# jonathanventura/spherical-sfm

Hardware: AMD Instinct MI355X
Metric: BA obs/sec (Jac+Schur+PCG) (higher is better)
Workload: dtype f64; 1 GPU; 300 cams x 100000 pts x 600000 obs synthetic circle (BASELINE configs[1]), general BA, focal fixed, CauchyLoss(1.0), Ceres-default LM; camera_dof=6, comm=none, reduced_solver=band-cholesky (direct), pcg_sweeps=0

## Files before the change

spherical_sfm_amd/csrc/ba_handle.h:

```cpp
#pragma once
#include <atomic>
#include <hip/hip_runtime.h>
#include <chrono>
#include <cmath>
#include <cstring>
#include <limits>
#include <string>
#include <vector>
#include "ba_flatten.h"
#include "ba_kernels.h"
#include "band_kernels2.h"
#include "band_kernels2p.h"
#include "band_sub.h"
#include "band_ring.h"
#include "snode.h"
#include "ssfm_ctx.h"
#include "knobs.h"

namespace ssfm {

static double wall_s() { return std::chrono::duration<double>(std::chrono::steady_clock::now().time_since_epoch()).count(); }

enum KernelId { KID_CAM_ROT, KID_POINT_LIN, KID_SCHUR_ROWS, KID_FINALIZE, KID_PCG_INIT, KID_PCG_MATVEC, KID_PCG_VECOPS,
                KID_CAM_UPDATE, KID_BACKSUB, KID_COST, KID_ALLREDUCE, KID_BAND_GATHER, KID_BAND_CHOL, KID_BAND_FWD, KID_BAND_BACK,
// ... 39 lines not shown

struct ssfm_ba_handle {
    ssfm_ctx* ctx = nullptr;
    int device = 0;
    ssfm_ba_options opt;
    BAFlat F;
    int n_red = 0;
    DevBuf<double> cam_x, cam_c, cam_init, pts_x, pts_c, pts_init, focal3;
    DevBuf<double> rot_x, rot_c, scale_cam, scale_pt, scale_f, mask_cam, mask_pt, mask_f, diag_cam, diag_pt, diag_f;
    DevBuf<double> obs_xy; DevBuf<int> obs_cam, obs_pt, pt_start, cam_start, cam_obs, row_ptr, col_idx, diag_slot;
    DevBuf<double> zone; bool zone_views = false; size_t zone_len = 0, zone_nnz = 0, zone_n = 0;
    bool det = false; DevBuf<long long> det_limb, det_lacc; DevBuf<double> det_dfpart; size_t det_nacc = 0;
    static constexpr size_t det_lacc_words = (size_t)SC_NSLOT * SC_TOTAL * LA_STRIDE;
    hipError_t clear_det_lacc() { return hipMemsetAsync(det_lacc.p, 0, det_lacc_words * sizeof(long long), ctx->stream); }
    void set_zone(int which) {
        scal.p = zone.p + (size_t)which * zone_len; pcg.p = scal.p + scal.n; redbuf.p = pcg.p + pcg.n;
        S_val = redbuf.p; rhs = S_val + zone_nnz; Udiag = rhs + (zone_n + 1); Sfc = Udiag + zone_n; gcraw = Sfc + zone_n; red_scal = gcraw + zone_n;
    }
    DevBuf<double> lmdev;
    DevBuf<double> Vs, gp, redbuf, Minv, Sff, px, pr, pz, pp, pq, pqpart, scal, pcg;
    DevBuf<double> band, Linv, Yb, Yr; DevBuf<int> cam_pos, band_pairs, band_fail, comp_ptr;
    BandSub sub; DevBuf<int> sub_seg_lo, sub_seg_hi, sub_seg_wend, sub_left, sub_sep_lo, sub_sep_rseg, sub_chain_ptr, sub_tw_lo, sub_tw_hi, sub_tw_copy, sub_seg_given, sub_seg_mode;
    DevBuf<unsigned char> pair_dummy;
    DevBuf<int> cam_pos2;
    DevBuf<double> subZ, subD, subT, subF, subL, subW, subC, subTc; DevBuf<int> sub_flags, sub_fz_lo, sub_fz_hi, sub_fz_wend, sub_fz_merge, sub_fz_await, sub_fz_signal, sub_fz_flags; int sub_seq = 0, sub_fz_seq = 0;
    DevBuf<int> col_pos, trans_pos;
    DevBuf<int> wrap_ptr, wrap_blk, wrap_row2, ring_rec, ring_tail; DevBuf<double> crL, crF, crW, crP, crT, crE;
    const int* wrap_ptr_p() const { return wrap_ptr.n ? wrap_ptr.p : nullptr; }
    SnodePlan sn; DevBuf<int> sn_half, sn_step, sn_node, sn_tab, sn_flags; DevBuf<double> sn_work, sn_xchg; int sn_seq = 0;
    DevBuf<int> trans_ptr, trans_blk, trans_row, pair_j, pair_j2, pair_p, batch_slot, cam_batch_ptr, chunk_cam, chunk_b0, chunk_b1, cam_obs_pt, cs_task_cam, cs_task_q0, cs_task_q1;
    double *S_val = nullptr, *rhs = nullptr, *Udiag = nullptr, *Sfc = nullptr, *gcraw = nullptr, *red_scal = nullptr;
    double focal_host = 0, t_flatten_s = 0;
    double* host_sp = nullptr;
    double* host_pub = nullptr;
    bool scale_ready = false;
    bool band_filled = false;
    struct { bool on = false, residual_later = false; const double *cam = nullptr, *focal = nullptr; double *cam_c = nullptr, *focal_c = nullptr, *rot_c = nullptr; } tail;
    DevBuf<int> gr_rec; DevBuf<unsigned char> pt_grouped;
    DevBuf<double> gram_part; DevBuf<int> gpart_off, fold_slot_ptr, fold_slot_src; bool gram_fold = false;
    DevBuf<int> pub_ticket;
    int pcg_prev_iters = 16;
    bool external_tail = false;
    bool profile = false;
    std::vector<hipEvent_t> ev_pool; size_t ev_used = 0;
    struct Span { int kid; hipEvent_t a, b; };
    std::vector<Span> spans;
    int64_t k_launches[KID_COUNT]; double k_ms[KID_COUNT];
    hipEvent_t phase_ev[5] = {nullptr, nullptr, nullptr, nullptr, nullptr};
    hipEvent_t x0_ev = nullptr;

    hipEvent_t get_event() {
        if (ev_used == ev_pool.size()) { hipEvent_t e; (void)hipEventCreate(&e); ev_pool.push_back(e); }
        return ev_pool[ev_used++];
    }
    void span_begin(int kid) { if (!profile) return; Span s{kid, get_event(), get_event()}; (void)hipEventRecord(s.a, ctx->stream); spans.push_back(s); }
    void span_end() { if (!profile) return; (void)hipEventRecord(spans.back().b, ctx->stream); }
    void resolve_spans() {
        for (auto& s : spans) { float ms = 0; if (hipEventElapsedTime(&ms, s.a, s.b) == hipSuccess) { k_ms[s.kid] += ms; k_launches[s.kid]++; } }
        spans.clear(); ev_used = 0;
    }
    void free_all() {
        cam_x.free(); cam_c.free(); cam_init.free(); pts_x.free(); pts_c.free(); pts_init.free(); focal3.free();
        rot_x.free(); rot_c.free(); scale_cam.free(); scale_pt.free(); scale_f.free(); mask_cam.free(); mask_pt.free(); mask_f.free();
        diag_cam.free(); diag_pt.free(); diag_f.free(); obs_xy.free(); obs_cam.free(); obs_pt.free(); pt_start.free();
        cam_start.free(); cam_obs.free(); row_ptr.free(); col_idx.free(); diag_slot.free(); Vs.free(); gp.free();
        lmdev.free(); band.free(); Linv.free(); Yb.free(); Yr.free(); cam_pos.free(); band_pairs.free(); band_fail.free(); comp_ptr.free();
        sub_seg_lo.free(); sub_seg_hi.free(); sub_seg_wend.free(); sub_left.free(); sub_sep_lo.free(); sub_sep_rseg.free(); sub_chain_ptr.free(); sub_tw_lo.free(); sub_tw_hi.free(); sub_tw_copy.free(); sub_seg_given.free(); sub_seg_mode.free(); cam_pos2.free(); pair_dummy.free();
        subZ.free(); subD.free(); subT.free(); subF.free(); subL.free(); subW.free(); subC.free(); subTc.free(); sub_flags.free(); sub_fz_lo.free(); sub_fz_hi.free(); sub_fz_wend.free(); sub_fz_merge.free(); sub_fz_await.free(); sub_fz_signal.free(); sub_fz_flags.free();
        col_pos.free(); trans_pos.free(); trans_ptr.free(); trans_blk.free(); trans_row.free(); pair_j.free(); pair_j2.free(); pair_p.free(); batch_slot.free(); cam_batch_ptr.free(); chunk_cam.free(); chunk_b0.free(); chunk_b1.free(); cam_obs_pt.free(); cs_task_cam.free(); cs_task_q0.free(); cs_task_q1.free();
        if (zone_views) { scal.p = nullptr; pcg.p = nullptr; redbuf.p = nullptr; zone_views = false; }
        pub_ticket.free(); gr_rec.free(); pt_grouped.free();
        gram_part.free(); gpart_off.free(); fold_slot_ptr.free(); fold_slot_src.free(); gram_fold = false;
        sn_half.free(); sn_step.free(); sn_node.free(); sn_tab.free(); sn_flags.free(); sn_work.free(); sn_xchg.free(); sn.enabled = false;
        wrap_ptr.free(); wrap_blk.free(); wrap_row2.free(); ring_rec.free(); ring_tail.free(); crL.free(); crF.free(); crW.free(); crP.free(); crT.free(); crE.free();
        zone.free(); redbuf.free(); Minv.free(); Sff.free(); px.free(); pr.free(); pz.free(); pp.free(); pq.free(); pqpart.free(); scal.free(); pcg.free();
        if (host_sp) { (void)hipHostFree(host_sp); host_sp = nullptr; }
        host_pub = nullptr;
        for (auto e : ev_pool) (void)hipEventDestroy(e);
        ev_pool.clear();
        for (auto& e : phase_ev) if (e) { (void)hipEventDestroy(e); e = nullptr; }
        if (x0_ev) { (void)hipEventDestroy(x0_ev); x0_ev = nullptr; }
    }
};

namespace ssfm {

#define MATVEC(h, DCV, vec)                                                                                                   \
    do {                                                                                                                   \
        if ((h)->F.sym_lower)                                                                                              \
            LAUNCH(h, KID_PCG_MATVEC, k_sym_matvec<DCV>, ((h)->F.Nc + 3) / 4, 256, 0, (h)->row_ptr.p, (h)->col_idx.p, (h)->trans_ptr.p, \
// ... 84 lines not shown
}
static int wait_published(ssfm_ba_handle* h) {
    ssfm_ctx* ctx = h->ctx;
    volatile unsigned long long* flag = reinterpret_cast<volatile unsigned long long*>(h->host_pub + SC_TOTAL + PCG_TOTAL + 1);
    const unsigned long long want = ctx->pub_seq;
    unsigned spins = 0;
    while (*flag != want) {
        cpu_relax();
        if ((++spins & 0xFFFFu) == 0) {
            const hipError_t q = hipStreamQuery(ctx->stream);
            if (q == hipSuccess) { if (*flag == want) break; return fail(ctx, SSFM_ERR_HIP, "an LM iteration ended without publishing its scalars"); }
            if (q != hipErrorNotReady) return fail(ctx, SSFM_ERR_HIP, hipGetErrorString(q));
        }
    }
    std::atomic_thread_fence(std::memory_order_acquire);
    return SSFM_OK;
}

static int sub_upload(ssfm_ba_handle* h, int DC) {
    ssfm_ctx* ctx = h->ctx; hipStream_t st = ctx->stream; const BAFlat& F = h->F;
    if (F.band_block > 0) DC = F.band_block;
    sub_build(F.comp_ptr, F.comp_twist, F.band, DC, h->sub, &F.rings);
    if (!F.wrap_ptr.empty()) { SSFM_HIP_CHECK(ctx, upload(h->wrap_ptr, F.wrap_ptr, st)); SSFM_HIP_CHECK(ctx, upload(h->wrap_blk, F.wrap_blk, st)); SSFM_HIP_CHECK(ctx, upload(h->wrap_row2, F.wrap_row2, st)); }
    if (!h->sub.enabled) return SSFM_OK;
    const BandSub& B = h->sub; const size_t Q = (size_t)F.band * DC, n = (size_t)(F.band_rows > 0 ? F.band_rows : F.Nc) * DC;
    SSFM_HIP_CHECK(ctx, upload(h->sub_tw_lo, B.tw_lo, st)); SSFM_HIP_CHECK(ctx, upload(h->sub_tw_hi, B.tw_hi, st)); SSFM_HIP_CHECK(ctx, upload(h->sub_tw_copy, B.tw_copy, st)); SSFM_HIP_CHECK(ctx, upload(h->sub_seg_given, B.seg_given, st));
    {
        std::vector<int> mode(B.seg_twist.size());
        for (size_t i = 0; i < mode.size(); i++) mode[i] = B.seg_twist[i] >= 0 ? 1 + (B.seg_twist[i] & 1) : 0;
        SSFM_HIP_CHECK(ctx, upload(h->sub_seg_mode, mode, st));
    }
    SSFM_HIP_CHECK(ctx, upload(h->sub_seg_lo, B.seg_lo, st)); SSFM_HIP_CHECK(ctx, upload(h->sub_seg_hi, B.seg_hi, st));
    SSFM_HIP_CHECK(ctx, upload(h->sub_seg_wend, B.seg_wend, st)); SSFM_HIP_CHECK(ctx, upload(h->sub_left, B.left_segs, st));
    SSFM_HIP_CHECK(ctx, upload(h->sub_sep_lo, B.sep_lo, st)); SSFM_HIP_CHECK(ctx, upload(h->sub_sep_rseg, B.sep_rseg, st));
    SSFM_HIP_CHECK(ctx, upload(h->sub_chain_ptr, B.chain_ptr, st));
    if (B.ntwist > 0) {
        SSFM_HIP_CHECK(ctx, upload(h->sub_fz_lo, B.fz_lo, st)); SSFM_HIP_CHECK(ctx, upload(h->sub_fz_hi, B.fz_hi, st)); SSFM_HIP_CHECK(ctx, upload(h->sub_fz_wend, B.fz_wend, st));
        SSFM_HIP_CHECK(ctx, upload(h->sub_fz_merge, B.fz_merge, st)); SSFM_HIP_CHECK(ctx, upload(h->sub_fz_await, B.fz_await, st)); SSFM_HIP_CHECK(ctx, upload(h->sub_fz_signal, B.fz_signal, st));
        SSFM_HIP_CHECK(ctx, h->sub_fz_flags.alloc((size_t)4 * B.ntwist)); SSFM_HIP_CHECK(ctx, hipMemsetAsync(h->sub_fz_flags.p, 0, (size_t)4 * B.ntwist * sizeof(int), st)); h->sub_fz_seq = 0;
    }
    if (B.nsep == 0) return SSFM_OK;
    SSFM_HIP_CHECK(ctx, h->subZ.alloc(Q * n)); SSFM_HIP_CHECK(ctx, h->subD.alloc((size_t)B.nsep * Q * Q)); SSFM_HIP_CHECK(ctx, h->subT.alloc((size_t)B.nsep * 2 * Q));
    SSFM_HIP_CHECK(ctx, h->subF.alloc((size_t)(B.nsep + B.nchain) * Q * Q)); SSFM_HIP_CHECK(ctx, h->subL.alloc((size_t)B.nsep * Q * (Q + 1) / 2)); SSFM_HIP_CHECK(ctx, h->subW.alloc((size_t)B.nsep * 2 * Q));
    SSFM_HIP_CHECK(ctx, h->subC.alloc((size_t)B.nchain * Q * (Q + 1) / 2)); SSFM_HIP_CHECK(ctx, h->subTc.alloc((size_t)B.nchain * 2 * Q)); SSFM_HIP_CHECK(ctx, h->sub_flags.alloc((size_t)2 * B.nchain));
    SSFM_HIP_CHECK(ctx, hipMemsetAsync(h->sub_flags.p, 0, (size_t)2 * B.nchain * sizeof(int), st)); h->sub_seq = 0;
    if (B.nring > 0) {
// ... 194 lines not shown
                    if (lb > 48 * 1024) SSFM_HIP_CHECK(ctx, hipFuncSetAttribute(reinterpret_cast<const void*>(k_ring_cr_back<DC, 2>), hipFuncAttributeMaxDynamicSharedMemorySize, (int)lb));
                    if (lt > 48 * 1024) SSFM_HIP_CHECK(ctx, hipFuncSetAttribute(reinterpret_cast<const void*>(k_ring_cr_tail<DC, 2>), hipFuncAttributeMaxDynamicSharedMemorySize, (int)lt));
                    const int nsteps = (int)B.ring_step_ptr.size() - 1;
                    const int cr_threads = Q > 48 ? 1024 : 512;
                    static int ring_stamp_state = SSFM_LAB_KNOB("SSFM_RING_STAMPS", 0) ? 1 : 0; static long long* ring_stamps = nullptr;
                    if (ring_stamp_state == 1) { (void)hipMalloc((void**)&ring_stamps, (size_t)4 * B.nsep * sizeof(long long)); (void)hipMemsetAsync(ring_stamps, 0, (size_t)4 * B.nsep * sizeof(long long), st); ring_stamp_state = 2; }
                    for (int sidx = 0; sidx < nsteps; sidx++)
                        LAUNCH(h, KID_RING_ELIM, (k_ring_cr_elim<DC, 2>), dim3(B.ring_step_ptr[sidx + 1] - B.ring_step_ptr[sidx], elim_roles(B.ring_step_ptr[sidx + 1] - B.ring_step_ptr[sidx])), cr_threads, le, h->ring_rec.p, B.ring_step_ptr[sidx], h->subZ.p, h->subD.p, h->subT.p,
                               h->crL.p, h->crF.p, h->crW.p, h->crP.p, h->crT.p, h->crE.p, Nc, b, failp, ring_stamp_state == 2 ? ring_stamps : (long long*)nullptr);
                    if (ring_stamp_state == 2) {
                        std::vector<long long> hs((size_t)4 * B.nsep); (void)hipStreamSynchronize(st); (void)hipMemcpy(hs.data(), ring_stamps, hs.size() * sizeof(long long), hipMemcpyDeviceToHost);
                        double a = 0, bb = 0, c = 0; int cnt = 0;
                        for (int q = 0; q < B.nsep; q++) if (hs[4 * q + 3] > 0) { a += hs[4 * q + 1] - hs[4 * q]; bb += hs[4 * q + 2] - hs[4 * q + 1]; c += hs[4 * q + 3] - hs[4 * q + 2]; cnt++; }
                        if (cnt) std::fprintf(stderr, "[ring stamps, 100 MHz ticks] Q = %d, %d eliminations (parallel steps): loads %.0f | factorisation %.0f | stores + neighbour products %.0f\n", Q, cnt, a / cnt, bb / cnt, c / cnt);
                        (void)hipFree(ring_stamps); ring_stamps = nullptr; ring_stamp_state = 3;
                    }
                    LAUNCH(h, KID_RING_TAIL, (k_ring_cr_tail<DC, 2>), B.nring, cr_threads, lt, h->ring_rec.p, h->ring_tail.p, h->subZ.p, h->subD.p, h->subT.p,
                           h->crL.p, h->crF.p, h->crW.p, h->crP.p, h->crT.p, h->crE.p, Y, Nc, b, failp);
                    for (int sidx = nsteps - 1; sidx >= 0; sidx--)
                        LAUNCH(h, KID_RING_BACK, (k_ring_cr_back<DC, 2>), B.ring_step_ptr[sidx + 1] - B.ring_step_ptr[sidx], back_threads, lb, h->ring_rec.p, B.ring_step_ptr[sidx], h->crL.p, h->crF.p, h->crW.p, Y, Nc, b);
                }
            }
            static const bool back_fuse = SSFM_LAB_KNOB("SSFM_BACK_FUSE", 0) != 0;
            if (B.ntwist > 0) {
                if (wide2p) SSFM_LAUNCH_CHOL2P(B.ntwist, h->sub_tw_lo.p, h->sub_tw_hi.p, h->sub_tw_hi.p, h->sub_tw_copy.p);
                else if (!fused) SSFM_LAUNCH_CHOL2(B.ntwist, h->band.p, h->Linv.p, Y, h->band_pairs.p, h->sub_tw_lo.p, h->sub_tw_hi.p, h->sub_tw_hi.p, h->sub_tw_copy.p, Nc, b, failp, chol_map);
                if (!back_fuse) {
                h->span_begin(KID_BAND_BACK);
                BACK_V2_LAUNCH(dim3(B.ntwist, 2), h->band.p, h->Linv.p, Y, h->sub_tw_lo.p, h->sub_tw_hi.p, h->sub_tw_hi.p, (const int*)nullptr, Nc, b);
                h->span_end();
                }
            }
            if (B.nleft > 0) {
                h->span_begin(KID_SUB_APPLY);
                hipLaunchKernelGGL((k_sub_apply_left<DC, 2>), dim3(B.nleft, (max_rows + APPLY_ROWS - 1) / APPLY_ROWS), dim3(APPLY_ROWS * APPLY_SLICES), (size_t)(2 * Q + APPLY_SLICES * APPLY_ROWS * 2) * sizeof(double), st, h->subZ.p, Y, h->sub_seg_lo.p, h->sub_seg_hi.p, h->sub_left.p, Nc, b);
                h->span_end();
            }
            h->span_begin(KID_BAND_BACK);
            BACK_V2_LAUNCH(dim3(B.nseg, 2), h->band.p, h->Linv.p, Y, h->sub_seg_lo.p, h->sub_seg_hi.p, h->sub_seg_wend.p, h->sub_seg_given.p, Nc, b, (const int*)(back_fuse ? h->sub_seg_mode.p : nullptr));
            h->span_end();
            return SSFM_OK;
        }
        if (wide2p) {
            SSFM_LAUNCH_CHOL2P(ncomp, h->comp_ptr.p, h->comp_ptr.p + 1, h->comp_ptr.p + 1, (const int*)nullptr);
            h->span_begin(KID_BAND_BACK);
            BACK_V2_LAUNCH(dim3(ncomp, 2), h->band.p, h->Linv.p, Y, h->comp_ptr.p, h->comp_ptr.p + 1, h->comp_ptr.p + 1, (const int*)nullptr, Nc, b);
            h->span_end();
        } else if (use_lds) {
            SSFM_LAUNCH_CHOL2(ncomp, h->band.p, h->Linv.p, Y, h->band_pairs.p, h->comp_ptr.p, h->comp_ptr.p + 1, h->comp_ptr.p + 1, (const int*)nullptr, Nc, b, reinterpret_cast<int*>(h->pcg.p + PCG_TOTAL), chol_map);
            if (back_v2) {
                h->span_begin(KID_BAND_BACK);
                BACK_V2_LAUNCH(dim3(ncomp, 2), h->band.p, h->Linv.p, Y, h->comp_ptr.p, h->comp_ptr.p + 1, h->comp_ptr.p + 1, (const int*)nullptr, Nc, b);
                h->span_end();
            } else {
                LAUNCH(h, KID_BAND_BACK, (k_band_back_lds<DC, 2>), ncomp, 256, lds_sub2, h->band.p, h->Linv.p, Y, h->comp_ptr.p, Nc, b);
            }
        } else {
            LAUNCH(h, KID_BAND_CHOL, (k_band_chol<DC, 2>), 1, 1024, lds_chol, h->band.p, h->Linv.p, Y, h->band_pairs.p, Nc, b, reinterpret_cast<int*>(h->pcg.p + PCG_TOTAL));
            LAUNCH(h, KID_BAND_BACK, (k_band_back<DC, 2>), 1, 256, lds_sub2, h->band.p, h->Linv.p, Y, Nc, b);
        }
        return SSFM_OK;
#undef SSFM_LAUNCH_CHOL2
#undef SSFM_LAUNCH_CHOL2_V
#undef SSFM_LAUNCH_CHOL2P
#undef SSFM_LAUNCH_2P
#undef SSFM_LAUNCH_2P6
    }

template <int DC>
static int band_resolve(ssfm_ba_handle* h, double* Y, bool* needs_refactor) {
    hipStream_t st = h->ctx->stream;
    const BAFlat& F = h->F;
// ... 114 lines not shown
```

spherical_sfm_amd/csrc/ba_solver.hip:

```cpp
#include <atomic>
#include <hip/hip_runtime.h>
#include <chrono>
#include <cmath>
#include <cstdlib>
#include <cstring>
#include <limits>
#include <string>
#include <vector>
#include "ba_flatten.h"
#include "ba_kernels.h"
#include "band_kernels.h"
#include "knobs.h"
#include "ssfm_ctx.h"

#include "ba_handle.h"

namespace ssfm {

constexpr unsigned DET_K_ASSEMBLY = (1u << SC_COST) | (1u << SC_FJJ) | (1u << SC_FJR) | (1u << SC_FWW) | (1u << SC_FWG);
constexpr unsigned DET_K_TAIL = (1u << SC_MODEL) | (1u << SC_STEP2_PT) | (1u << SC_XN2_PT) | (1u << SC_CAND_COST) | (1u << SC_STEP2_CAM) | (1u << SC_XN2_CAM);
static unsigned det_tail_mask(bool with_cams, bool gram_fold) {
    const unsigned tail = with_cams ? (DET_K_TAIL & ~((1u << SC_STEP2_CAM) | (1u << SC_XN2_CAM))) : DET_K_TAIL;
    return tail | (gram_fold ? (1u << SC_COST) : 0u);
}
// ... 62 lines not shown
            double* host_sp = h->host_sp;
            for (int k = 0; k < SC_TOTAL; k++) {
                double a = host_sp[k];
                for (int s2 = 1; s2 < SC_NSLOT; s2++) { const double v = host_sp[(size_t)s2 * SC_TOTAL + k]; a = (k == SC_GMAX) ? std::max(a, v) : a + v; }
                host_sp[k] = a;
            }
        }
        return SSFM_OK;
    }
    int need_x0() {
        if (!x0_pending) return SSFM_OK;
        SSFM_HIP_CHECK(ctx, hipEventSynchronize(h->x0_ev));
        x_norm = std::sqrt(host_scal[SC_X0N2_PT] + host_scal[SC_X0N2_CAM]); x0_pending = false;
        return SSFM_OK;
    }

    int read_knobs() {
        poll = lm_poll() && publish_alloc(h);
        if (!poll && !h->host_sp) SSFM_HIP_CHECK(ctx, hipHostMalloc((void**)&h->host_sp, (SC_NSLOT * SC_TOTAL + PCG_TOTAL + 1) * sizeof(double), hipHostMallocDefault));
        host_scal = poll ? h->host_pub : h->host_sp; host_pcg1 = poll ? h->host_pub + SC_TOTAL : h->host_sp + SC_NSLOT * SC_TOTAL;
        spec_on = poll && nP > 0 && knob_env_int("SSFM_LM_SPECULATE", 1) != 0;
        gram_bs = knob_env_int("SSFM_GRAM_BACKSUB", -1);
        gbs_split_env = knob_env_int("SSFM_GBS_SPLIT", 0);
        fuse_lin = SSFM_LAB_KNOB("SSFM_GRAM_FUSE", 0) != 0 && nP > 0 && !F.gr_rec.empty() && F.gram_points == (int64_t)nP && F.chunk_cam.empty() && F.cs_task_cam.empty();
        return SSFM_OK;
    }

    int startup() {
        { const int rc = read_knobs(); if (rc) return rc; }
        const int gp_pts = (nP + 255) / 256;
        h->set_zone(0);
        if (h->det) {
            if (!h->gram_fold) SSFM_HIP_CHECK(ctx, hipMemsetAsync(h->det_limb.p, 0, (2 * h->det_nacc + 2) * sizeof(long long), st));
            SSFM_HIP_CHECK(ctx, h->clear_det_lacc());
        }
        const bool make_scale = !h->scale_ready;
        LAUNCH(h, KID_CAM_ROT, k_cam_rot0, gp_cam, 64, 0, x.cam, x.rot, Nc, h->scal.p, (int)SC_TOTAL, h->diag_f.p, make_scale ? 1 : 0);
        if (make_scale) {
            if (nP > 0) hipLaunchKernelGGL(k_colnorm_both, dim3(gp_pts + Nc), dim3(256), 0, st, gp_pts, x.cam, x.rot, x.pts, x.focal, oxy, h->obs_cam.p, h->pt_start.p, nP,
                                           loss, la, h->diag_pt.p, h->diag_f.p, h->mask_pt.p, h->scale_pt.p, O.jacobi_scaling, h->det ? h->det_dfpart.p : (double*)nullptr,
                                           h->obs_pt.p, h->cam_start.p, h->cam_obs.p, h->diag_cam.p, h->mask_cam.p, ctx->collective ? (double*)nullptr : h->scale_cam.p);
            else hipLaunchKernelGGL(k_colnorm_cam, dim3(Nc), dim3(256), 0, st, x.cam, x.rot, x.pts, x.focal, oxy, h->obs_pt.p, h->cam_start.p, h->cam_obs.p,
                               loss, la, h->diag_cam.p, h->mask_cam.p, ctx->collective ? (double*)nullptr : h->scale_cam.p, O.jacobi_scaling);
            if (ctx->collective) {
                int rc = allreduce(h, h->diag_cam.p, (size_t)Nc * 6, ncclSum); if (rc) return rc;
                rc = allreduce(h, h->diag_f.p, 1, ncclSum); if (rc) return rc;
// ... 378 lines not shown
}

extern "C" int ssfm_band_solve_probe(ssfm_ctx* ctx, int32_t dc, int32_t N, int32_t b, int32_t ncomp, const int32_t* comp_ptr, const double* band,
                                     double* Y, int32_t* segs_seps_fail, double* Zdump, double* Ddump, double* Tdump) {
    if (!ctx || (dc != 3 && dc != 6) || N <= 0 || b < 1 || ncomp < 1 || !comp_ptr || !band || !Y) return fail(ctx, SSFM_ERR_INVALID, "ssfm_band_solve_probe: bad arguments");
    SSFM_HIP_CHECK(ctx, hipSetDevice(ctx->device));
    hipStream_t st = ctx->stream;
    ssfm_ba_handle hh; ssfm_ba_handle* h = &hh;
    h->ctx = ctx; ssfm_ba_default_options(&h->opt);
    std::memset(h->k_launches, 0, sizeof(h->k_launches)); std::memset(h->k_ms, 0, sizeof(h->k_ms));
    BAFlat& F = h->F; F.Nc = N; F.band_rows = N; F.band_block = dc; F.band = b; F.DC = dc; F.comp_ptr.assign(comp_ptr, comp_ptr + ncomp + 1);
    for (int ir = 1; ir <= b; ir++) for (int kr = 1; kr <= ir; kr++) F.band_pairs.push_back(ir | (kr << 16));
    const size_t nb = (size_t)N * (b + 1) * dc * dc, n = (size_t)N * dc;
    int rc = SSFM_OK;
    auto run = [&]() -> int {
        SSFM_HIP_CHECK(ctx, h->band.alloc(nb)); SSFM_HIP_CHECK(ctx, h->Linv.alloc((size_t)N * dc * dc)); SSFM_HIP_CHECK(ctx, h->Yb.alloc(2 * n));
        SSFM_HIP_CHECK(ctx, h->pcg.alloc(PCG_TOTAL + 1));
        SSFM_HIP_CHECK(ctx, hipMemsetAsync(h->pcg.p, 0, (PCG_TOTAL + 1) * sizeof(double), st));
        SSFM_HIP_CHECK(ctx, hipMemsetAsync(h->Linv.p, 0, (size_t)N * dc * dc * sizeof(double), st));
        SSFM_HIP_CHECK(ctx, hipMemcpyAsync(h->band.p, band, nb * sizeof(double), hipMemcpyHostToDevice, st));
        SSFM_HIP_CHECK(ctx, hipMemcpyAsync(h->Yb.p, Y, 2 * n * sizeof(double), hipMemcpyHostToDevice, st));
        SSFM_HIP_CHECK(ctx, upload(h->band_pairs, F.band_pairs, st)); SSFM_HIP_CHECK(ctx, upload(h->comp_ptr, F.comp_ptr, st));
        { const int r = sub_upload(h, dc); if (r) return r; }
        if (h->sub.enabled && h->subZ.p) SSFM_HIP_CHECK(ctx, hipMemsetAsync(h->subZ.p, 0, h->subZ.n * sizeof(double), st));
        { const int r = (dc == 3) ? band_direct<3>(h, h->Yb.p) : band_direct<6>(h, h->Yb.p); if (r) return r; }
        SSFM_HIP_CHECK(ctx, hipMemcpyAsync(Y, h->Yb.p, 2 * n * sizeof(double), hipMemcpyDeviceToHost, st));
        int flag = 0;
        SSFM_HIP_CHECK(ctx, hipMemcpyAsync(&flag, h->pcg.p + PCG_TOTAL, sizeof(int), hipMemcpyDeviceToHost, st));
        if (h->sub.enabled) {
            if (Zdump) SSFM_HIP_CHECK(ctx, hipMemcpyAsync(Zdump, h->subZ.p, h->subZ.n * sizeof(double), hipMemcpyDeviceToHost, st));
            if (Ddump) SSFM_HIP_CHECK(ctx, hipMemcpyAsync(Ddump, h->subD.p, h->subD.n * sizeof(double), hipMemcpyDeviceToHost, st));
            if (Tdump) SSFM_HIP_CHECK(ctx, hipMemcpyAsync(Tdump, h->subT.p, h->subT.n * sizeof(double), hipMemcpyDeviceToHost, st));
        }
        SSFM_HIP_CHECK(ctx, hipStreamSynchronize(st));
        if (segs_seps_fail) { segs_seps_fail[0] = h->sub.enabled ? h->sub.nseg : ncomp; segs_seps_fail[1] = h->sub.nsep; segs_seps_fail[2] = flag; }
        return SSFM_OK;
    };
    rc = run();
    h->free_all();
    return rc;
}


extern "C" int ssfm_snode_solve_probe(ssfm_ctx* ctx, int32_t dc, int32_t Nc, const int32_t* row_ptr, const int32_t* col_idx, const double* S_val, const double* rhs2,
                                      int32_t nr, double* Y, int32_t* info) {
    if (!ctx || (dc != 3 && dc != 6) || Nc <= 0 || !row_ptr || !col_idx || !S_val || !rhs2 || !Y || !info || (nr != 1 && nr != 2)) return fail(ctx, SSFM_ERR_INVALID, "ssfm_snode_solve_probe: bad arguments");
// ... 507 lines not shown
```

spherical_sfm_amd/csrc/band_kernels2.h:

```cpp
#pragma once
#include <type_traits>
#include "band_kernels.h"

namespace ssfm {

__device__ __forceinline__ double lane_bcast(double v, int src_lane) {
    const int lo = __builtin_amdgcn_readlane(__double2loint(v), src_lane), hi = __builtin_amdgcn_readlane(__double2hiint(v), src_lane);
    return __hiloint2double(hi, lo);
}
__device__ __forceinline__ double lane_shift_down(double v, int delta) {
    const int idx = (int)(((threadIdx.x & 63) + delta) & 63) << 2;
    const int lo = __builtin_amdgcn_ds_bpermute(idx, __double2loint(v)), hi = __builtin_amdgcn_ds_bpermute(idx, __double2hiint(v));
    return __hiloint2double(hi, lo);
}

template <int DC>
__device__ __forceinline__ bool wave_chol_inverse(double (&row)[DC], double (&g)[DC]) {
    const int lane = threadIdx.x & 63;
    double L[DC], rs[DC]; bool ok = true;
#pragma unroll
    for (int c = 0; c < DC; c++) {
        double d = lane_bcast(row[c], c);
        ok = ok && (d > 0.0);
        rs[c] = fast_rsqrt(d);
// ... 19 lines not shown
    if (nw != 9) return m;
    int weight[16], order[16];
    for (int r = 0; r < nw; r++) {
        weight[r] = (r == 0) ? 12 : (r <= ntw) ? ((r <= heavy_tw) ? 6 : 2) : (r == nw - 1) ? 5 : 4;
        order[r] = r;
    }
    for (int a = 0; a < nw; a++) for (int c = a + 1; c < nw; c++) if (weight[order[c]] > weight[order[a]]) { const int t = order[a]; order[a] = order[c]; order[c] = t; }
    int load[4] = {0, 0, 0, 0}, used[4] = {0, 0, 0, 0}, cap[4];
    for (int q = 0; q < 4; q++) cap[q] = (nw - q + 3) / 4;
    bool placed[16] = {false};
    m.v[0] = (unsigned char)order[0]; placed[0] = true; used[0] = 1;
    for (int a = nw - 1; a >= 1 && used[0] < cap[0]; a--) { m.v[4 * used[0]] = (unsigned char)order[a]; placed[a] = true; used[0]++; }
    for (int a = 1; a < nw; a++) {
        if (placed[a]) continue;
        int best = -1;
        for (int q = 1; q < 4; q++) if (used[q] < cap[q] && (best < 0 || load[q] < load[best])) best = q;
        m.v[best + 4 * used[best]] = (unsigned char)order[a];
        load[best] += weight[order[a]]; used[best]++;
    }
    return m;
}

constexpr int BACK_PD = 4;
template <int DC, int NS, bool to_lds, bool from_lds>
__device__ __forceinline__ void band_back_sweep(const double* __restrict__ band, const double* __restrict__ Ginv, double* __restrict__ y, double* xs,
                                                const int r0, const int r1, const int re, const int gf, const int b, const int lane) {
    constexpr int BB = DC * DC;
    const int W = b + 1, T = b * DC;
    int dd[NS], off[NS]; bool has[NS];
#pragma unroll
    for (int s = 0; s < NS; s++) {
        const int t = min(lane + 64 * s, T - 1);
        dd[s] = t / DC + 1; off[s] = dd[s] * BB + (t - (dd[s] - 1) * DC); has[s] = lane + 64 * s < T;
    }
    const int lc = min(lane, DC - 1);
    struct Stage { double col[NS][DC], li[DC], yv; };
    const size_t row_stride = (size_t)W * BB;
        Stage st[BACK_PD];
        auto fetch = [&](int j, Stage& s) {
            const int jc = max(j, r0);
            const double* __restrict__ rowp = band + (size_t)jc * row_stride;
            const double* __restrict__ gpt = Ginv + (size_t)jc * BB;
#pragma unroll
            for (int m = 0; m < DC; m++) {
#pragma unroll
                for (int q = 0; q < NS; q++) s.col[q][m] = rowp[off[q] + m * DC];
                s.li[m] = gpt[m * DC + lc];
            }
            const int jy = (gf >= 0 && jc >= r1) ? gf + (re - 1 - jc) : jc;
            s.yv = (from_lds && jc >= r1) ? xs[(jy - gf) * DC + lc] : y[(size_t)jy * DC + lc];
        };
#pragma unroll
        for (int u = 0; u < BACK_PD; u++) fetch(re - 1 - u, st[u]);
        double acc[NS];
#pragma unroll
        for (int q = 0; q < NS; q++) acc[q] = 0.0;
        for (int jb = re - 1; jb >= r0; jb -= BACK_PD) {
#pragma unroll
            for (int u = 0; u < BACK_PD; u++) {
                const int j = jb - u;
                if (j < r0) break;
                double c[NS][DC], cl[DC]; const double cy = st[u].yv;
                bool v[NS];
#pragma unroll
                for (int q = 0; q < NS; q++) v[q] = has[q] && j - dd[q] >= r0;
#pragma unroll
                for (int m = 0; m < DC; m++) {
#pragma unroll
                    for (int q = 0; q < NS; q++) c[q][m] = st[u].col[q][m];
                    cl[m] = st[u].li[m];
                }
                fetch(j - BACK_PD, st[u]);
                const double z = cy - acc[0];
                double sh[NS], sft[NS];
#pragma unroll
                for (int q = 0; q < NS; q++) sh[q] = lane_shift_down(acc[q], DC);
#pragma unroll
                for (int q = 0; q < NS; q++) {
                    const double next = (q + 1 < NS) ? sh[q + 1 < NS ? q + 1 : q] : 0.0;
                    sft[q] = (lane + DC < 64) ? sh[q] : next;
                    if (!(lane + 64 * q + DC < T)) sft[q] = 0.0;
                }
                double x = 0.0;
#pragma unroll
                for (int k = 0; k < DC; k++) x += cl[k] * lane_bcast(z, k);
                if (j >= r1) x = cy;
                else if (lane < DC) { if (to_lds) xs[(j - r0) * DC + lane] = x; else y[(size_t)j * DC + lane] = x; }
                double sm[NS];
#pragma unroll
                for (int q = 0; q < NS; q++) sm[q] = 0.0;
#pragma unroll
                for (int m = 0; m < DC; m++) { const double xm = lane_bcast(x, m);
#pragma unroll
                    for (int q = 0; q < NS; q++) sm[q] += c[q][m] * xm; }
#pragma unroll
                for (int q = 0; q < NS; q++) acc[q] = sft[q] + (v[q] ? sm[q] : 0.0);
            }
        }
}

template <int DC, int NR, int MF = 0, int TCW = 3>
__global__ void __launch_bounds__(768)
k_band_chol_v2(double* __restrict__ band, double* __restrict__ Ginv, double* __restrict__ Y, const int* __restrict__ pairs,
               const int* __restrict__ piv_lo, const int* __restrict__ piv_hi, const int* __restrict__ win_hi,
               const int* __restrict__ merge_from, int N, int b, int* __restrict__ fail_flag,
               const CholWaveMap wmap,
               const int* __restrict__ await2 = nullptr, const int* __restrict__ signal = nullptr, int* __restrict__ flags = nullptr, int seq = 0) {
    constexpr int BB = DC * DC;
    extern __shared__ __attribute__((aligned(16))) double lds[];
    const int R = b + 1, W = b + 1, RW = W * BB;
    double* sWin = lds;
    double* sP = sWin + (size_t)R * RW;
    double* sYr = sP + (size_t)b * BB;
    double* sYj = sYr + (size_t)R * NR * DC;
    double* sG = sYj + NR * DC;
    double* sD = sG + BB;
    int* sPairs = reinterpret_cast<int*>(sD + BB);
    const int n = N * DC, nt = blockDim.x, lane = threadIdx.x & 63, nw = nt >> 6;
    const int wave = __builtin_amdgcn_readfirstlane((int)wmap.v[threadIdx.x >> 6]), tid = wave * 64 + lane;
    const int ntw = nw - 2 - CHOL2_LOADERS;
    const int r0 = piv_lo[blockIdx.x], r1 = piv_hi[blockIdx.x], re = win_hi[blockIdx.x];
    const int sig = signal ? signal[blockIdx.x] : -1, aw = await2 ? await2[blockIdx.x] : -1;
    if (r0 >= r1) { if (sig >= 0 && tid == 0) __hip_atomic_store(flags + sig, seq, __ATOMIC_RELEASE, __HIP_MEMORY_SCOPE_AGENT); return; }
    for (int e = tid; e < b * (b + 1) / 2; e += nt) sPairs[e] = pairs[e];
    if (aw >= 0) {
        if (tid == 0) { while (__hip_atomic_load(flags + aw, __ATOMIC_ACQUIRE, __HIP_MEMORY_SCOPE_AGENT) != seq) __builtin_amdgcn_s_sleep(8);
                        while (__hip_atomic_load(flags + aw + 1, __ATOMIC_ACQUIRE, __HIP_MEMORY_SCOPE_AGENT) != seq) __builtin_amdgcn_s_sleep(8); }
        __syncthreads(); __threadfence();
    }
    const int mf = merge_from ? merge_from[blockIdx.x] : -1;
// ... 363 lines not shown
#undef CHOL2_ISSUE
#undef CHOL2_STEP
    } else {
        int jm = jm0;
        for (int j = r0; j < r1; j++, jm = (jm + 1 == R) ? 0 : jm + 1) {
            const int nb = min(b, re - 1 - j);
            phaseB(j, jm, nb);
            for (int e = lane; e < BB; e += 64) Ginv[(size_t)j * BB + e] = sG[e];
            lds_barrier();
            for (int e = lane; e < nb * BB; e += 64) { const int k = e / BB; band[((size_t)(j + 1 + k) * W + (k + 1)) * BB + (e - k * BB)] = sP[e]; }
            if (lane < NR * DC) Y[(size_t)(lane / DC) * n + (size_t)j * DC + (lane % DC)] = sYj[lane];
            lds_barrier();
        }
    }
    if (re > r1) {
        __syncthreads();
        for (int row = r1; row < re; row++) {
            const int nin = (row - r1 + 1) * BB;
            const double* src = sWin + (size_t)(row % R) * RW;
            for (int e = tid; e < nin; e += nt) band[(size_t)row * RW + e] = src[e];
            for (int e = tid; e < NR * DC; e += nt) Y[(size_t)(e / DC) * n + (size_t)row * DC + (e % DC)] = sYr[(size_t)(row % R) * NR * DC + e];
        }
    }
    if (sig >= 0) {
        __threadfence(); __syncthreads();
        if (tid == 0) __hip_atomic_store(flags + sig, seq, __ATOMIC_RELEASE, __HIP_MEMORY_SCOPE_AGENT);
    }
}

template <int DC, int NS>
__global__ void __launch_bounds__(64)
k_band_back_v2(const double* __restrict__ band, const double* __restrict__ Ginv, double* __restrict__ Y, const int* __restrict__ piv_lo,
               const int* __restrict__ piv_hi, const int* __restrict__ win_hi, const int* __restrict__ given_from, int N, int b,
               const int* __restrict__ tw_mode = nullptr) {
    __shared__ double xs[32 * DC];
    const int n = N * DC, lane = threadIdx.x;
    const int mode = tw_mode ? tw_mode[blockIdx.x] : 0;
    if (piv_lo[blockIdx.x] >= piv_hi[blockIdx.x]) return;
    double* y = Y + (size_t)blockIdx.y * n;
    const int r0 = piv_lo[blockIdx.x], r1 = piv_hi[blockIdx.x], re = win_hi[blockIdx.x];
    const int gf = given_from ? given_from[blockIdx.x] : -1;
    if (mode == 2) {
        band_back_sweep<DC, NS, true, false>(band, Ginv, y, xs, gf, gf + b, gf + b, -1, b, lane);
        __builtin_amdgcn_fence(__ATOMIC_RELEASE, "wavefront"); __builtin_amdgcn_fence(__ATOMIC_ACQUIRE, "wavefront");
        band_back_sweep<DC, NS, false, true>(band, Ginv, y, xs, r0, r1, re, gf, b, lane);
    } else band_back_sweep<DC, NS, false, false>(band, Ginv, y, xs, r0, mode == 1 ? re : r1, re, mode == 1 ? -1 : gf, b, lane);
// ... 4 lines not shown
```

spherical_sfm_amd/csrc/rotavg_solver.hip:

```cpp
#include <algorithm>
#include <cstdio>
#include "ba_handle.h"
#include "dual.h"
#include "line_search.h"

namespace ssfm {

struct EdgeConst { double meas[9]; double r[3]; double rx, ry, thetaxy, thetaz; };

static void decompose_rotation_host(const double* R, double& rx, double& ry, double& thetaxy, double& thetaz) {
    double Z[3] = {R[2], R[5], R[8]};
    const double zn = norm3(Z); Z[0] /= zn; Z[1] /= zn; Z[2] /= zn;
    const double axis[3] = {-Z[1], Z[0], 0.0};
    const double an = norm3(axis);
    const double rxy[3] = {axis[0] / an, axis[1] / an, axis[2] / an};
    thetaxy = acos(Z[2]);
    const double v[3] = {thetaxy * rxy[0], thetaxy * rxy[1], thetaxy * rxy[2]};
    double Rxy[9]; so3exp(v, Rxy);
    rx = rxy[0]; ry = rxy[1];
    double Rz[9]; mat3_mul_at(Rxy, R, Rz);
    double rz[3]; so3ln(Rz, rz);
    thetaz = rz[2];
}

// ... 574 lines not shown
        }
        std::vector<int> nptr(n + 1, 0), nedge, nslot; std::vector<unsigned char> nside, nfirst;
        for (int i = 0; i < n; i++) {
            auto& v = adj[i];
            std::sort(v.begin(), v.end(), [](const Ent& p, const Ent& q) { return p.nb != q.nb ? p.nb < q.nb : p.e < q.e; });
            for (size_t k = 0; k < v.size(); k++) {
                nedge.push_back(v[k].e); nside.push_back(v[k].side);
                nslot.push_back((int)(std::lower_bound(F.col_idx.begin() + F.row_ptr[i], F.col_idx.begin() + F.row_ptr[i + 1], v[k].nb) - (F.col_idx.begin() + F.row_ptr[i])));
                nfirst.push_back((k == 0 || v[k - 1].nb != v[k].nb) ? 1 : 0);
            }
            nptr[i + 1] = (int)nedge.size();
        }
        if (nedge.empty()) { nedge.push_back(0); nslot.push_back(0); nside.push_back(0); nfirst.push_back(0); }
        std::vector<int> zero2(2, 0);
        SSFM_HIP_CHECK(ctx, su.up(RS.nadj_ptr, nptr)); SSFM_HIP_CHECK(ctx, su.up(RS.nadj_edge, nedge)); SSFM_HIP_CHECK(ctx, su.up(RS.nadj_slot, nslot));
        SSFM_HIP_CHECK(ctx, su.up(RS.nadj_side, nside)); SSFM_HIP_CHECK(ctx, su.up(RS.nadj_first, nfirst)); SSFM_HIP_CHECK(ctx, su.up(RS.ticket, zero2));
        ALV(RS.ejac, (size_t)24 * E); ALV(RS.node_part, (size_t)3 * ((E + 63) / 64)); ALV(RS.wg_part, (size_t)5 * ((E + 63) / 64 + gnode)); ALV(RS.step_part, (size_t)5 * 32);
    }
#undef ALV
    double* fmx = fm2.p; double* fmc = fm2.p + 1; double* xx = x.p; double* xcand = xc.p;
    const int ge = (E + 63) / 64, gn = (n + 63) / 64;
    const double la = O.loss_scale;
    const bool poll = lm_poll() && publish_alloc(h);
    if (!poll && !h->host_sp) SSFM_HIP_CHECK(ctx, hipHostMalloc((void**)&h->host_sp, (SC_NSLOT * SC_TOTAL + PCG_TOTAL + 1) * sizeof(double), hipHostMallocDefault));
    double* host_scal = poll ? h->host_pub : h->host_sp; double* host_pcg = poll ? h->host_pub + SC_TOTAL : h->host_sp + SC_NSLOT * SC_TOTAL;
    SSFM_HIP_CHECK(ctx, hipMemsetAsync(h->zone.p, 0, h->zone.n * sizeof(double), st));
    auto assemble = [&](const double* s3, const double* sf) -> int {
        if (node_major) {
            hipLaunchKernelGGL(k_rot_edge_records, dim3(ge), dim3(64), 0, st, kind, E, e0.p, e1.p, ec.p, G.scale, la, xx, fmx, s3, sf, RS.ejac.p, RS.node_part.p);
            hipLaunchKernelGGL(k_rot_gather_nodes, dim3(n), dim3(64), 0, st, n, ge, RS.nadj_ptr.p, RS.nadj_edge.p, RS.nadj_side.p, RS.nadj_slot.p, RS.nadj_first.p, RS.ejac.p, RS.node_part.p,
                               h->row_ptr.p, h->diag_slot.p, h->S_val, h->rhs, h->Udiag, h->Sfc, h->scal.p, h->pcg.p + PCG_TOTAL);
        } else
        hipLaunchKernelGGL(k_rot_edges, dim3(ge), dim3(64), 0, st, 0, kind, E, e0.p, e1.p, ec.p, G.scale, la, xx, fmx, s3, sf, h->row_ptr.p, h->col_idx.p, n,
                           (const double*)nullptr, h->S_val, h->rhs, h->Udiag, h->Sfc, h->scal.p);
        return SSFM_OK;
    };
    {
        DevBuf<double>&m3 = RS.m3, &mf = RS.mf; std::vector<double> mfv = {with_f ? 1.0 : 0.0};
        SSFM_HIP_CHECK(ctx, su.up(m3, G.mask)); SSFM_HIP_CHECK(ctx, su.up(mf, mfv));
        int rc = assemble(m3.p, mf.p); if (rc) return rc;
        hipLaunchKernelGGL(k_make_scale, dim3((3 * n + 255) / 256), dim3(256), 0, st, h->Udiag, m3.p, sc3.p, 3 * n, O.jacobi_scaling);
        hipLaunchKernelGGL(k_make_scale, dim3(1), dim3(64), 0, st, h->scal.p + SC_FJJ, mf.p, scf.p, 1, O.jacobi_scaling);
        hipLaunchKernelGGL(k_scale3to6, dim3((6 * n + 255) / 256), dim3(256), 0, st, sc3.p, n, sc6.p);
        if (timing) SSFM_HIP_CHECK(ctx, hipStreamSynchronize(st));
    }
    lap("allocations, uploads, Jacobi scaling");
// ... 154 lines not shown
```

Baseline: 3.565 billion obs/s.

## Fuse band back-substitution into the Cholesky kernel tail

Adds a per-component or per-twist record table and runs the banded back-substitution sweeps at the end of the LDS Cholesky kernel, instead of launching a separate back-sweep kernel. Idle waves prefetch the band and Ginv segments into cache while the main sweep runs, and the back sweep uses a configurable prefetch depth. This removes one kernel launch and the band re-read from the per-LM-iteration direct solve. In exchange it adds extra barriers and a serial back sweep inside the Cholesky workgroup, and it only applies under specific segment layouts.

```diff
diff --git a/spherical_sfm_amd/csrc/ba_handle.h b/spherical_sfm_amd/csrc/ba_handle.h
--- a/spherical_sfm_amd/csrc/ba_handle.h
+++ b/spherical_sfm_amd/csrc/ba_handle.h
@@ -85,6 +85,7 @@
     DevBuf<double> band, Linv, Yb, Yr; DevBuf<int> cam_pos, band_pairs, band_fail, comp_ptr;
     BandSub sub; DevBuf<int> sub_seg_lo, sub_seg_hi, sub_seg_wend, sub_left, sub_sep_lo, sub_sep_rseg, sub_chain_ptr, sub_tw_lo, sub_tw_hi, sub_tw_copy, sub_seg_given, sub_seg_mode;
     DevBuf<unsigned char> pair_dummy;
+    DevBuf<int> back_rec; bool back_in_chol = true;
     DevBuf<int> cam_pos2;
     DevBuf<double> subZ, subD, subT, subF, subL, subW, subC, subTc; DevBuf<int> sub_flags, sub_fz_lo, sub_fz_hi, sub_fz_wend, sub_fz_merge, sub_fz_await, sub_fz_signal, sub_fz_flags; int sub_seq = 0, sub_fz_seq = 0;
     DevBuf<int> col_pos, trans_pos;
@@ -128,7 +129,7 @@
         diag_cam.free(); diag_pt.free(); diag_f.free(); obs_xy.free(); obs_cam.free(); obs_pt.free(); pt_start.free();
         cam_start.free(); cam_obs.free(); row_ptr.free(); col_idx.free(); diag_slot.free(); Vs.free(); gp.free();
         lmdev.free(); band.free(); Linv.free(); Yb.free(); Yr.free(); cam_pos.free(); band_pairs.free(); band_fail.free(); comp_ptr.free();
-        sub_seg_lo.free(); sub_seg_hi.free(); sub_seg_wend.free(); sub_left.free(); sub_sep_lo.free(); sub_sep_rseg.free(); sub_chain_ptr.free(); sub_tw_lo.free(); sub_tw_hi.free(); sub_tw_copy.free(); sub_seg_given.free(); sub_seg_mode.free(); cam_pos2.free(); pair_dummy.free();
+        sub_seg_lo.free(); sub_seg_hi.free(); sub_seg_wend.free(); sub_left.free(); sub_sep_lo.free(); sub_sep_rseg.free(); sub_chain_ptr.free(); sub_tw_lo.free(); sub_tw_hi.free(); sub_tw_copy.free(); sub_seg_given.free(); sub_seg_mode.free(); back_rec.free(); cam_pos2.free(); pair_dummy.free();
         subZ.free(); subD.free(); subT.free(); subF.free(); subL.free(); subW.free(); subC.free(); subTc.free(); sub_flags.free(); sub_fz_lo.free(); sub_fz_hi.free(); sub_fz_wend.free(); sub_fz_merge.free(); sub_fz_await.free(); sub_fz_signal.free(); sub_fz_flags.free();
         col_pos.free(); trans_pos.free(); trans_ptr.free(); trans_blk.free(); trans_row.free(); pair_j.free(); pair_j2.free(); pair_p.free(); batch_slot.free(); cam_batch_ptr.free(); chunk_cam.free(); chunk_b0.free(); chunk_b1.free(); cam_obs_pt.free(); cs_task_cam.free(); cs_task_q0.free(); cs_task_q1.free();
         if (zone_views) { scal.p = nullptr; pcg.p = nullptr; redbuf.p = nullptr; zone_views = false; }
@@ -259,6 +260,16 @@
     if (F.band_block > 0) DC = F.band_block;
     sub_build(F.comp_ptr, F.comp_twist, F.band, DC, h->sub, &F.rings);
     if (!F.wrap_ptr.empty()) { SSFM_HIP_CHECK(ctx, upload(h->wrap_ptr, F.wrap_ptr, st)); SSFM_HIP_CHECK(ctx, upload(h->wrap_blk, F.wrap_blk, st)); SSFM_HIP_CHECK(ctx, upload(h->wrap_row2, F.wrap_row2, st)); }
+    {
+        const BandSub& Bs = h->sub;
+        const int nrec = Bs.enabled ? Bs.ntwist : (int)F.comp_ptr.size() - 1;
+        std::vector<int> rec((size_t)BACK_REC_INTS * std::max(nrec, 0), 0);
+        if (Bs.enabled) for (int sg = 0; sg < Bs.nseg; sg++) if (Bs.seg_twist[sg] >= 0) {
+            int* r = rec.data() + (size_t)BACK_REC_INTS * (Bs.seg_twist[sg] >> 1) + 4 * (Bs.seg_twist[sg] & 1);
+            r[0] = Bs.seg_lo[sg]; r[1] = Bs.seg_hi[sg]; r[2] = Bs.seg_wend[sg]; r[3] = Bs.seg_given[sg];
+        }
+        if (nrec > 0) SSFM_HIP_CHECK(ctx, upload(h->back_rec, rec, st));
+    }
     if (!h->sub.enabled) return SSFM_OK;
     const BandSub& B = h->sub; const size_t Q = (size_t)F.band * DC, n = (size_t)(F.band_rows > 0 ? F.band_rows : F.Nc) * DC;
     SSFM_HIP_CHECK(ctx, upload(h->sub_tw_lo, B.tw_lo, st)); SSFM_HIP_CHECK(ctx, upload(h->sub_tw_hi, B.tw_hi, st)); SSFM_HIP_CHECK(ctx, upload(h->sub_tw_copy, B.tw_copy, st)); SSFM_HIP_CHECK(ctx, upload(h->sub_seg_given, B.seg_given, st));
@@ -499,6 +510,12 @@
                 }
             }
             static const bool back_fuse = SSFM_LAB_KNOB("SSFM_BACK_FUSE", 0) != 0;
+            const bool back_in = h->back_in_chol && b * DC <= 64 && !wide2p && !fused && !back_fuse && B.ntwist > 0 && B.nsep == 0 && B.nleft == 0 && B.nseg == 2 * B.ntwist && h->back_rec.p;
+            if (back_in) {
+                SSFM_LAUNCH_CHOL2(B.ntwist, h->band.p, h->Linv.p, Y, h->band_pairs.p, h->sub_tw_lo.p, h->sub_tw_hi.p, h->sub_tw_hi.p, h->sub_tw_copy.p, Nc, b, failp, chol_map,
+                                  (const int*)nullptr, (const int*)nullptr, (int*)nullptr, 0, (const int*)h->back_rec.p);
+                return SSFM_OK;
+            }
             if (B.ntwist > 0) {
                 if (wide2p) SSFM_LAUNCH_CHOL2P(B.ntwist, h->sub_tw_lo.p, h->sub_tw_hi.p, h->sub_tw_hi.p, h->sub_tw_copy.p);
                 else if (!fused) SSFM_LAUNCH_CHOL2(B.ntwist, h->band.p, h->Linv.p, Y, h->band_pairs.p, h->sub_tw_lo.p, h->sub_tw_hi.p, h->sub_tw_hi.p, h->sub_tw_copy.p, Nc, b, failp, chol_map);
@@ -524,7 +541,10 @@
             BACK_V2_LAUNCH(dim3(ncomp, 2), h->band.p, h->Linv.p, Y, h->comp_ptr.p, h->comp_ptr.p + 1, h->comp_ptr.p + 1, (const int*)nullptr, Nc, b);
             h->span_end();
         } else if (use_lds) {
-            SSFM_LAUNCH_CHOL2(ncomp, h->band.p, h->Linv.p, Y, h->band_pairs.p, h->comp_ptr.p, h->comp_ptr.p + 1, h->comp_ptr.p + 1, (const int*)nullptr, Nc, b, reinterpret_cast<int*>(h->pcg.p + PCG_TOTAL), chol_map);
+            const bool back_in = h->back_in_chol && back_v2 && b * DC <= 64 && h->back_rec.p && (int)h->back_rec.n == BACK_REC_INTS * ncomp;
+            SSFM_LAUNCH_CHOL2(ncomp, h->band.p, h->Linv.p, Y, h->band_pairs.p, h->comp_ptr.p, h->comp_ptr.p + 1, h->comp_ptr.p + 1, (const int*)nullptr, Nc, b, reinterpret_cast<int*>(h->pcg.p + PCG_TOTAL), chol_map,
+                              (const int*)nullptr, (const int*)nullptr, (int*)nullptr, 0, (const int*)(back_in ? h->back_rec.p : nullptr));
+            if (back_in) return SSFM_OK;
             if (back_v2) {
                 h->span_begin(KID_BAND_BACK);
                 BACK_V2_LAUNCH(dim3(ncomp, 2), h->band.p, h->Linv.p, Y, h->comp_ptr.p, h->comp_ptr.p + 1, h->comp_ptr.p + 1, (const int*)nullptr, Nc, b);
diff --git a/spherical_sfm_amd/csrc/ba_solver.hip b/spherical_sfm_amd/csrc/ba_solver.hip
--- a/spherical_sfm_amd/csrc/ba_solver.hip
+++ b/spherical_sfm_amd/csrc/ba_solver.hip
@@ -108,6 +108,7 @@
         spec_on = poll && nP > 0 && knob_env_int("SSFM_LM_SPECULATE", 1) != 0;
         gram_bs = knob_env_int("SSFM_GRAM_BACKSUB", -1);
         gbs_split_env = knob_env_int("SSFM_GBS_SPLIT", 0);
+        h->back_in_chol = knob_env_int("SSFM_BAND_BACK_IN_CHOL", 1) != 0;
         fuse_lin = SSFM_LAB_KNOB("SSFM_GRAM_FUSE", 0) != 0 && nP > 0 && !F.gr_rec.empty() && F.gram_points == (int64_t)nP && F.chunk_cam.empty() && F.cs_task_cam.empty();
         return SSFM_OK;
     }
@@ -532,6 +533,7 @@
         SSFM_HIP_CHECK(ctx, hipMemcpyAsync(h->Yb.p, Y, 2 * n * sizeof(double), hipMemcpyHostToDevice, st));
         SSFM_HIP_CHECK(ctx, upload(h->band_pairs, F.band_pairs, st)); SSFM_HIP_CHECK(ctx, upload(h->comp_ptr, F.comp_ptr, st));
         { const int r = sub_upload(h, dc); if (r) return r; }
+        h->back_in_chol = knob_env_int("SSFM_BAND_BACK_IN_CHOL", 1) != 0;
         if (h->sub.enabled && h->subZ.p) SSFM_HIP_CHECK(ctx, hipMemsetAsync(h->subZ.p, 0, h->subZ.n * sizeof(double), st));
         { const int r = (dc == 3) ? band_direct<3>(h, h->Yb.p) : band_direct<6>(h, h->Yb.p); if (r) return r; }
         SSFM_HIP_CHECK(ctx, hipMemcpyAsync(Y, h->Yb.p, 2 * n * sizeof(double), hipMemcpyDeviceToHost, st));
diff --git a/spherical_sfm_amd/csrc/band_kernels2.h b/spherical_sfm_amd/csrc/band_kernels2.h
--- a/spherical_sfm_amd/csrc/band_kernels2.h
+++ b/spherical_sfm_amd/csrc/band_kernels2.h
@@ -65,7 +65,7 @@
 }
 
 constexpr int BACK_PD = 4;
-template <int DC, int NS, bool to_lds, bool from_lds>
+template <int DC, int NS, bool to_lds, bool from_lds, int PD = BACK_PD>
 __device__ __forceinline__ void band_back_sweep(const double* __restrict__ band, const double* __restrict__ Ginv, double* __restrict__ y, double* xs,
                                                 const int r0, const int r1, const int re, const int gf, const int b, const int lane) {
     constexpr int BB = DC * DC;
@@ -79,7 +79,7 @@
     const int lc = min(lane, DC - 1);
     struct Stage { double col[NS][DC], li[DC], yv; };
     const size_t row_stride = (size_t)W * BB;
-        Stage st[BACK_PD];
+        Stage st[PD];
         auto fetch = [&](int j, Stage& s) {
             const int jc = max(j, r0);
             const double* __restrict__ rowp = band + (size_t)jc * row_stride;
@@ -94,13 +94,13 @@
             s.yv = (from_lds && jc >= r1) ? xs[(jy - gf) * DC + lc] : y[(size_t)jy * DC + lc];
         };
 #pragma unroll
-        for (int u = 0; u < BACK_PD; u++) fetch(re - 1 - u, st[u]);
+        for (int u = 0; u < PD; u++) fetch(re - 1 - u, st[u]);
         double acc[NS];
 #pragma unroll
         for (int q = 0; q < NS; q++) acc[q] = 0.0;
-        for (int jb = re - 1; jb >= r0; jb -= BACK_PD) {
-#pragma unroll
-            for (int u = 0; u < BACK_PD; u++) {
+        for (int jb = re - 1; jb >= r0; jb -= PD) {
+#pragma unroll
+            for (int u = 0; u < PD; u++) {
                 const int j = jb - u;
                 if (j < r0) break;
                 double c[NS][DC], cl[DC]; const double cy = st[u].yv;
@@ -113,7 +113,7 @@
                     for (int q = 0; q < NS; q++) c[q][m] = st[u].col[q][m];
                     cl[m] = st[u].li[m];
                 }
-                fetch(j - BACK_PD, st[u]);
+                fetch(j - PD, st[u]);
                 const double z = cy - acc[0];
                 double sh[NS], sft[NS];
 #pragma unroll
@@ -140,6 +140,48 @@
                 for (int q = 0; q < NS; q++) acc[q] = sft[q] + (v[q] ? sm[q] : 0.0);
             }
         }
+}
+
+struct BackRec { int seg[2][4]; };
+constexpr int BACK_REC_INTS = 8;
+static_assert(sizeof(BackRec) == BACK_REC_INTS * sizeof(int), "BackRec is uploaded as a table of ints");
+
+template <int DC, int NS, int NR>
+__device__ __forceinline__ void band_back_in_chol(const double* band, const double* Ginv, double* Y, const int* __restrict__ rec, const int r0, const int r1,
+                                               const int n, const int b, const int wave, const int nw, const int lane) {
+#ifndef SSFM_CPD
+#define SSFM_CPD 2
+#endif
+    constexpr int CPD = DC > 3 ? SSFM_CPD : BACK_PD;
+    static_assert(2 * NR <= 3 + CHOL2_LOADERS, "a workgroup has at least 3 + CHOL2_LOADERS waves: one per sweep");
+    __builtin_amdgcn_fence(__ATOMIC_RELEASE, "workgroup"); __syncthreads(); __builtin_amdgcn_fence(__ATOMIC_ACQUIRE, "workgroup");
+    int seg[2][4];
+#pragma unroll
+    for (int q = 0; q < 8; q++) seg[q >> 2][q & 3] = __builtin_amdgcn_readfirstlane(rec[q]);
+    if (wave < NR) band_back_sweep<DC, NS, false, false, CPD>(band, Ginv, Y + (size_t)wave * n, nullptr, r0, r1, r1, -1, b, lane);
+    else {
+        constexpr int BB = DC * DC;
+        const int W = b + 1, nl = (nw - NR) * 64, l0 = (wave - NR) * 64 + lane;
+#pragma unroll
+        for (int q = 0; q < 2; q++) {
+            if (seg[q][0] >= seg[q][1]) continue;
+            const char* pb = reinterpret_cast<const char*>(band + (size_t)seg[q][0] * W * BB); const long nb_ = (long)(seg[q][1] - seg[q][0]) * W * BB * 8;
+            const char* pg = reinterpret_cast<const char*>(Ginv + (size_t)seg[q][0] * BB); const long ng_ = (long)(seg[q][1] - seg[q][0]) * BB * 8;
+            for (long o = (long)l0 * 128; o < nb_ + ng_; o += (long)nl * 128 * 4) {
+                int t0, t1, t2, t3;
+                const long o1 = o + (long)nl * 128, o2 = o1 + (long)nl * 128, o3 = o2 + (long)nl * 128, last = nb_ + ng_ - 4;
+                auto at = [&](long x) { x = x < last ? x : last; return x < nb_ ? pb + x : pg + (x - nb_); };
+                const char *a0 = at(o), *a1 = at(o1), *a2 = at(o2), *a3 = at(o3);
+                asm volatile("global_load_dword %0, %4, off\n\tglobal_load_dword %1, %5, off\n\tglobal_load_dword %2, %6, off\n\tglobal_load_dword %3, %7, off\n\ts_waitcnt vmcnt(0)"
+                             : "=&v"(t0), "=&v"(t1), "=&v"(t2), "=&v"(t3) : "v"(a0), "v"(a1), "v"(a2), "v"(a3) : "memory");
+            }
+        }
+    }
+    __builtin_amdgcn_fence(__ATOMIC_RELEASE, "workgroup"); __syncthreads(); __builtin_amdgcn_fence(__ATOMIC_ACQUIRE, "workgroup");
+    if (wave < 2 * NR) {
+        const int q = wave / NR, lo = seg[q][0], hi = seg[q][1], we = seg[q][2], gf = seg[q][3];
+        if (lo < hi) band_back_sweep<DC, NS, false, false, CPD>(band, Ginv, Y + (size_t)(wave % NR) * n, nullptr, lo, hi, we, gf, b, lane);
+    }
 }
 
 template <int DC, int NR, int MF = 0, int TCW = 3>
@@ -148,7 +190,8 @@
                const int* __restrict__ piv_lo, const int* __restrict__ piv_hi, const int* __restrict__ win_hi,
                const int* __restrict__ merge_from, int N, int b, int* __restrict__ fail_flag,
                const CholWaveMap wmap,
-               const int* __restrict__ await2 = nullptr, const int* __restrict__ signal = nullptr, int* __restrict__ flags = nullptr, int seq = 0) {
+               const int* __restrict__ await2 = nullptr, const int* __restrict__ signal = nullptr, int* __restrict__ flags = nullptr, int seq = 0,
+               const int* __restrict__ back_rec = nullptr) {
     constexpr int BB = DC * DC;
     extern __shared__ __attribute__((aligned(16))) double lds[];
     const int R = b + 1, W = b + 1, RW = W * BB;
@@ -558,6 +601,9 @@
             for (int e = tid; e < NR * DC; e += nt) Y[(size_t)(e / DC) * n + (size_t)row * DC + (e % DC)] = sYr[(size_t)(row % R) * NR * DC + e];
         }
     }
+    if (back_rec) {
+        band_back_in_chol<DC, 1, NR>(band, Ginv, Y, back_rec + (size_t)BACK_REC_INTS * blockIdx.x, r0, r1, n, b, wave, nw, lane);
+    }
     if (sig >= 0) {
         __threadfence(); __syncthreads();
         if (tid == 0) __hip_atomic_store(flags + sig, seq, __ATOMIC_RELEASE, __HIP_MEMORY_SCOPE_AGENT);
diff --git a/spherical_sfm_amd/csrc/rotavg_solver.hip b/spherical_sfm_amd/csrc/rotavg_solver.hip
--- a/spherical_sfm_amd/csrc/rotavg_solver.hip
+++ b/spherical_sfm_amd/csrc/rotavg_solver.hip
@@ -620,6 +620,7 @@
     const int ge = (E + 63) / 64, gn = (n + 63) / 64;
     const double la = O.loss_scale;
     const bool poll = lm_poll() && publish_alloc(h);
+    h->back_in_chol = knob_env_int("SSFM_BAND_BACK_IN_CHOL", 1) != 0;
     if (!poll && !h->host_sp) SSFM_HIP_CHECK(ctx, hipHostMalloc((void**)&h->host_sp, (SC_NSLOT * SC_TOTAL + PCG_TOTAL + 1) * sizeof(double), hipHostMallocDefault));
     double* host_scal = poll ? h->host_pub : h->host_sp; double* host_pcg = poll ? h->host_pub + SC_TOTAL : h->host_sp + SC_NSLOT * SC_TOTAL;
     SSFM_HIP_CHECK(ctx, hipMemsetAsync(h->zone.p, 0, h->zone.n * sizeof(double), st));
```

Result: slower. 3.301 billion obs/s (-7.4%).
